# NJU-3DV/Relightable3DGaussian

Measured on AMD Instinct MI355X. Metric: train iters/s, synthetic lego-like 800x800, 300000 Gaussians (stage-2 hot path), higher is better.
Workload: dtype f32; 1 GPU; stage-2 train iteration (fused glue kernels + one-launch Adam): shading fwd/bwd (K=64) + rasterize fwd (S=16) + loss + rasterize bwd + Adam; 1 view/rank/step, 300000 Gaussians, 800x800, num_rendered~1755024; parallelism=dp1

## Files before the change

### relightable3dgaussian_amd/csrc/capi_shading.hip

```cpp
#include "capi_internal.hpp"

using namespace r3dg;

extern "C" {

int r3dg_shade_forward_cached(void* stream_, int P, int K, int M, const float* base_color, const float* roughness,
                              const float* normals, const float* viewdirs, const float* incidents, const float* env,
                              int He, int We, const float* env_transform, const float* visibility,
                              const float* incident_dirs, const float* incident_areas, float uniform_area,
                              const uint32_t* taps, int flags, float* out)
{
    if (P < 0 || K <= 0 || He <= 0 || We <= 0) return invalid("shade_forward: bad P/K/env size");
    if (He > 32767 || We > 32767) return invalid("shade_forward: environment map larger than 32767 texels per side");
    if (M != 1 && M != 4 && M != 9 && M != 16) return invalid("shade_forward: incidents must hold 1, 4, 9 or 16 SH coefficients");
    if (P == 0) return R3DG_OK;
    if (!base_color || !roughness || !normals || !viewdirs || !incidents || !env || !visibility || !incident_dirs || !out)
        return invalid("shade_forward: null buffer");
    return guarded([&]() -> int {
        hipStream_t stream = (hipStream_t)stream_;
        StageTimer t(stream, ST_SHADE_FWD);
        launch_shade_forward(stream, P, K, M, base_color, roughness, normals, viewdirs, incidents, env, He, We,
                             env_transform, visibility, incident_dirs, incident_areas, out, taps,
                             (flags & R3DG_SHADE_TRAIN_OUTPUTS) != 0, uniform_area, (flags & R3DG_SHADE_TAPS_ARE_RADIANCE) != 0,
                             (flags & R3DG_SHADE_LEAVE_ROOM) != 0);
// ... 239 lines not shown
    if (!shade_frs_supported(K, 16, He, We))
        return invalid("shade_frs_backward: needs K % 4 == 0 and an environment texture that fits LDS (r3dg_shade_frs_supported)");
    if (P == 0) return R3DG_OK;
    if (!base_color || !roughness || !normals || !viewdirs || !incidents || !env || !visibility || !taps || !ray_normals ||
        !zsamples || !tables || !valid || !cprime || !dcprime || !dL_dpbr || !dL_ddiffuse_light || !dL_dbase_color ||
        !dL_droughness || !dL_dviewdirs || !dL_dincidents || !dL_denv || (n_invalid > 0 && !invalid_list))
        return invalid("shade_frs_backward: null buffer");
    return guarded([&]() -> int {
        hipStream_t stream = (hipStream_t)stream_;
        int gmax_n = 1;
        const unsigned int* gmax;
        {
            StageTimer t(stream, ST_SHADE_AUX);
            gmax = launch_shade_frs_backward_aux(stream, P, dL_dpbr, dL_ddiffuse_light, block_absmax, n_block_absmax, &gmax_n);
        }
        if (n_invalid > 0) {
            StageTimer t(stream, ST_SHADE_LISTED);
            launch_shade_frs_backward_listed(stream, K, base_color, roughness, normals, viewdirs, incidents, env, He, We,
                                             visibility, ray_normals, zsamples, uniform_area, invalid_list, n_invalid, dL_dpbr,
                                             dL_ddiffuse_light, dL_dbase_color, dL_droughness, dL_dviewdirs, dL_dincidents,
                                             dL_denv, gmax, gmax_n);
        }
        {
            StageTimer t(stream, ST_SHADE_BWD);
            launch_shade_frs_backward_main(stream, P, K, base_color, roughness, normals, viewdirs, env, He, We, visibility,
                                           uniform_area, taps, ray_normals, tables, valid, cprime, dcprime, dL_dpbr,
                                           dL_ddiffuse_light, dL_dbase_color, dL_droughness, dL_dviewdirs, dL_denv, gmax, gmax_n);
        }
        if (no_rotation_back) return R3DG_OK;
        hipStream_t rstream = rotate_stream_ != nullptr ? (hipStream_t)rotate_stream_ : stream;
        stream_wait_stream(rstream, stream);
        {
            StageTimer t(rstream, ST_SHADE_AUX);
            launch_shade_frs_backward_rotate(rstream, P, ray_normals, dcprime, dL_dincidents, n_invalid > 0 ? valid : nullptr);
        }
        return R3DG_OK;
    });
}

int r3dg_shade_frs_incident_chain(void* stream_, int P, const float* ray_normals, const uint8_t* valid, const float* dcprime,
                                  float* dL_dincidents, float* incidents, float* exp_avg, float* exp_avg_sq, float* cprime,
                                  float lr, float lr_tail, float beta1, float beta2, float eps, int step, float grad_scale,
// ... 100 lines not shown
```

### relightable3dgaussian_amd/csrc/launchers.hpp

```cpp
#pragma once
#include "common.hpp"

namespace r3dg {

constexpr int REFILL_MIN_IDLE = 16;

void release_gradient_records();
void launch_mark_visible(hipStream_t s, int P, const float* means3D, const float* vm, uint8_t* present);
void launch_preprocess(hipStream_t s, int P, int D, int M, const float* means3D, const float* scales, float scale_modifier,
                       const float* rotations, const float* opacities, const float* shs, uint8_t* clamped,
                       const float* cov3D_precomp, const float* colors_precomp, const float* vm, const float* pm,
                       const float* cam_pos, int W, int H, float tan_fovx, float tan_fovy, float focal_x, float focal_y,
                       int* radii, float* means2D, float* depths, float* cov3Ds, float* rgb, float* conic_opacity,
                       float* splat, int gx, int gy, uint32_t* tiles_touched, uint32_t* block_sums,
                       unsigned long long* total, bool scan_now, uint32_t* zero_words, int zero_n);
void launch_duplicate_with_keys(hipStream_t s, int P, const float* means2D, const float* depths,
                                const uint32_t* tiles_touched, const uint32_t* block_offsets, uint32_t* point_offsets,
                                uint64_t* keys, uint32_t* values, const int* radii, int gx, int gy);
void launch_identify_tile_ranges(hipStream_t s, int L, const uint64_t* keys, uint32_t* ranges);
void launch_tile_order(hipStream_t s, int T, const uint32_t* ranges, uint32_t* order, uint32_t small_cap, uint32_t* big_list,
                       uint32_t* big_count);
void launch_render_forward(hipStream_t s, int W, int H, int S, const uint32_t* tile_order, const uint32_t* ranges,
                           const uint32_t* point_list, const float* splat, const float* features, float* final_T,
                           uint32_t* n_contrib, const float* bg, float* out_color, float* out_opacity, float* out_depth,
// ... 33 lines not shown
                                   const float* visibility, float uniform_area, const uint32_t* taps,
                                   const float* ray_normals, const float* tables, const uint8_t* valid, const float* cprime,
                                   bool leave_room, float* out, float* feat);
void launch_shade_frs_forward_listed(hipStream_t s, int K, const float* base_color, const float* roughness,
                                     const float* normals, const float* viewdirs, const float* incidents, const float* env,
                                     int He, int We, const float* visibility, const float* ray_normals,
                                     const float* zsamples, float uniform_area, const int* invalid_list, int n_invalid,
                                     float* out, float* feat);
void launch_shade_frs_incident_chain(hipStream_t s, int P, const float* ray_normals, const uint8_t* valid, const float* dcp,
                                     float* d_inc, float* incidents, float* exp_avg, float* exp_avg_sq, float* cprime,
                                     float lr, float lr_tail, float beta1, float beta2, float eps, int step,
                                     float grad_scale, const float* skip_flag, int listed_in_dcprime);
const unsigned int* launch_shade_frs_backward_aux(hipStream_t s, int P, const float* g_pbr, const float* g_diff,
                                                  const float* block_absmax, int n_block_absmax, int* gmax_n);
void launch_shade_frs_backward_main(hipStream_t s, int P, int K, const float* base_color, const float* roughness,
                                    const float* normals, const float* viewdirs, const float* env, int He, int We,
                                    const float* visibility, float uniform_area, const uint32_t* taps,
                                    const float* ray_normals, const float* tables, const uint8_t* valid, const float* cprime,
                                    float* dcp, const float* g_pbr, const float* g_diff, float* d_base, float* d_rough,
                                    float* d_view, float* d_env, const unsigned int* gmax, int gmax_n);
void launch_shade_frs_backward_rotate(hipStream_t s, int P, const float* ray_normals, const float* dcp, float* d_inc,
                                      const uint8_t* valid);
void launch_shade_frs_backward_listed(hipStream_t s, int K, const float* base_color, const float* roughness,
                                      const float* normals, const float* viewdirs, const float* incidents, const float* env,
                                      int He, int We, const float* visibility, const float* ray_normals,
                                      const float* zsamples, float uniform_area, const int* invalid_list, int n_invalid,
                                      const float* g_pbr, const float* g_diff, float* d_base, float* d_rough, float* d_view,
                                      float* d_inc, float* d_env, const unsigned int* gmax, int gmax_n);
void launch_shade_build_taps(hipStream_t s, size_t n, const float* dirs, const float* tr, int He, int We, const float* env,
                             uint32_t* taps);
void launch_shade_build_split(hipStream_t s, int P, int K, const int* perm, const float* normals, const float* incidents,
                              const float* visibility, const float* dirs, const float* zsamples, float uniform_area,
                              float* lt, float* vis_t, float* consts);
void launch_shade_forward_split(hipStream_t s, int P, int K, const int* perm, const float* base_color,
                                const float* roughness, const float* normals, const float* viewdirs, const float* lt,
                                const float* vis_t, const float* consts, const float* zsamples, const float* tr,
                                const float* env4, int He, int We, float* out);
void launch_shade_env_footprints(hipStream_t s, int He, int We, const float* env, float* fp);
void launch_shade_build_transport(hipStream_t s, int P, int K, int M, const float* normals, const float* incidents,
                                  const float* visibility, const float* dirs, const float* areas, float uniform_area,
                                  float* radiance_to_transport, float* consts);
void launch_shade_forward_transport(hipStream_t s, int P, int K, const float* base_color, const float* roughness,
                                    const float* normals, const float* viewdirs, const float* transport, const float* consts,
// ... 123 lines not shown
```

### relightable3dgaussian_amd/csrc/shading.hip

```cpp
#include "launchers.hpp"
#include <cmath>
#include <cstdlib>
#include <map>
#include <mutex>
#include <stdexcept>
#include <tuple>
#include "wave_reduce.hpp"
#include "shading_math.hpp"

namespace r3dg {

constexpr int SHADE_WAVES = 4;
constexpr int ENV_LDS_MAX = 12288;

__device__ __forceinline__ float fast_acosf(float x)
{
    const float ax = fabsf(x);
    const bool big = ax > 0.5f;
    const float z = big ? 0.5f * (1.0f - ax) : x * x;
    const float s = big ? sqrtf(z) : ax;
    float p = 4.2163199048e-2f;
    p = p * z + 2.4181311049e-2f;
    p = p * z + 4.5470025998e-2f;
    p = p * z + 7.4953002686e-2f;
// ... 100 lines not shown
            o.idx[a * 2 + b] = ok ? __mul24(y, We) + x : -1;
            o.w[a * 2 + b] = wy[a] * wx[b];
        }
    return o;
}

struct SampleFwd {
    float local[3], glob[3], lin[3], transport[3];
    float spec, ndi, area_ndi;
    float Y[16], shsum[3];
    float L[3], Hh[3], ulen, NoL, NoH, VoH, rawNoH, rawVoH, nom0, nom1, nom2, nomr, frac0, p2;
    EnvTap taps;
    float vis;
};

template <bool ENV_LDS, bool HAVE_SHSUM = false, bool HAVE_TAP = false>
__device__ __forceinline__ void shade_sample(SampleFwd& s, const GaussFwd& G, const float* sh ,
                                             int M, float dx, float dy, float dz, float vis, float area,
                                             const float* __restrict__ env, const float* s_env,
                                             const float* __restrict__ tr, int He, int We, const PackedTap* cached = nullptr)
{
    if (HAVE_TAP) s.taps = taps_from_packed(*cached, He, We);
    else s.taps = env_taps(dx, dy, dz, tr, He, We);
    s.vis = vis;
    float e[3] = {0.f, 0.f, 0.f};
#pragma unroll
    for (int t = 0; t < 4; t++) {
        if (s.taps.idx[t] >= 0) {
            float3 px;
            if (ENV_LDS) {
                const float* q = s_env + 3 * s.taps.idx[t];
                px = make_float3(q[0], q[1], q[2]);
            } else {
                px = *reinterpret_cast<const float3*>(env + 3 * (size_t)s.taps.idx[t]);
            }
            e[0] += px.x * s.taps.w[t];
            e[1] += px.y * s.taps.w[t];
            e[2] += px.z * s.taps.w[t];
        }
    }
    {
        float acc[3];
        if (HAVE_SHSUM) {
            acc[0] = s.shsum[0]; acc[1] = s.shsum[1]; acc[2] = s.shsum[2];
        } else {
            sh_basis16(dx, dy, dz, M, s.Y);
// ... 947 lines not shown
{
    unsigned int* scratch = shade_scratch();
    const unsigned int* gmax = scratch;
    *gmax_n = 1;
    if (block_absmax != nullptr && n_block_absmax > 0) {
        gmax = reinterpret_cast<const unsigned int*>(block_absmax);
        *gmax_n = n_block_absmax;
    } else {
        R3DG_HIP(hipMemsetAsync(scratch, 0, 4, s));
        const int nb = (3 * P + 255) / 256;
        grad_absmax_kernel<<<nb < 256 ? nb : 256, 256, 0, s>>>(3 * P, g_pbr, g_diff, scratch);
    }
    return gmax;
}

void launch_shade_frs_backward_main(hipStream_t s, int P, int K, const float* base_color, const float* roughness,
                                    const float* normals, const float* viewdirs, const float* env, int He, int We,
                                    const float* visibility, float uniform_area, const uint32_t* taps, const float* ray_normals,
                                    const float* tables, const uint8_t* valid, const float* cprime, float* dcp, const float* g_pbr,
                                    const float* g_diff, float* d_base, float* d_rough, float* d_view, float* d_env,
                                    const unsigned int* gmax, int gmax_n)
{
    if (P == 0) return;
    const bool tab_lds = K <= FRS_TAB_LDS_MAX_K;
    const size_t smem = frs_backward_lds_bytes(K, He, We);
    const FrsSrc src = {base_color, roughness, normals, viewdirs, ray_normals, cprime, g_pbr, g_diff, visibility, taps};
    if (tab_lds) {
        const int grid = frs_grid(P, (const void*)shade_backward_frs_kernel<true>, smem);
        shade_backward_frs_kernel<true><<<grid, 64 * FRS_WAVES, smem, s>>>(
            P, K, src, env, He, We, frs_area(uniform_area), tables, valid, d_base, d_rough, d_view, dcp, d_env, gmax, gmax_n);
    } else {
        const int grid = frs_grid(P, (const void*)shade_backward_frs_kernel<false>, smem);
        shade_backward_frs_kernel<false><<<grid, 64 * FRS_WAVES, smem, s>>>(
            P, K, src, env, He, We, frs_area(uniform_area), tables, valid, d_base, d_rough, d_view, dcp, d_env, gmax, gmax_n);
    }
    check_launch(s, false, "shade_backward_frs_kernel");
}

void launch_shade_frs_backward_rotate(hipStream_t s, int P, const float* ray_normals, const float* dcp, float* d_inc,
                                      const uint8_t* valid)
{
    if (P == 0) return;
    frs_rotate_kernel<true><<<(P + 255) / 256, 256, 0, s>>>(P, ray_normals, dcp, d_inc, valid);
    check_launch(s, false, "frs_rotate_kernel");
}

void launch_shade_frs_incident_chain(hipStream_t s, int P, const float* ray_normals, const uint8_t* valid, const float* dcp,
                                     float* d_inc, float* incidents, float* exp_avg, float* exp_avg_sq, float* cprime, float lr,
                                     float lr_tail, float beta1, float beta2, float eps, int step, float grad_scale,
                                     const float* skip_flag, int listed_in_dcprime)
{
    if (P == 0) return;
    const double b1 = 1.0 - pow((double)beta1, (double)step), b2 = 1.0 - pow((double)beta2, (double)step);
    FrsAdam a = {lr, lr_tail, beta1, beta2, eps, (float)b1, (float)(1.0 / sqrt(b2)), grad_scale, 1.f - beta1, 1.f - beta2};
    const size_t lds = 4 * 64 * FRS_CHAIN_LD * sizeof(float);
    frs_incident_chain_kernel<<<(P + 255) / 256, 256, lds, s>>>(P, ray_normals, valid, dcp, d_inc, incidents, exp_avg, exp_avg_sq,
                                                                cprime, a, skip_flag, listed_in_dcprime);
    check_launch(s, false, "frs_incident_chain_kernel");
}

void launch_shade_frs_backward_listed(hipStream_t s, int K, const float* base_color, const float* roughness,
                                      const float* normals, const float* viewdirs, const float* incidents, const float* env, int He,
                                      int We, const float* visibility, const float* ray_normals, const float* zsamples,
                                      float uniform_area, const int* invalid_list, int n_invalid, const float* g_pbr,
                                      const float* g_diff, float* d_base, float* d_rough, float* d_view, float* d_inc, float* d_env,
                                      const unsigned int* gmax, int gmax_n)
{
    if (n_invalid <= 0) return;
    const FrsSrc src = {base_color, roughness, normals, viewdirs, ray_normals, nullptr, g_pbr, g_diff, visibility, nullptr};
    const size_t smem = (3 * (((size_t)3 * He * We + 3) & ~(size_t)3) + 64 * FRS_LISTED_WAVES) * sizeof(float);
    int grid = frs_listed_grid(n_invalid);
    grid = grid > 64 ? 64 + (grid - 64) / 4 : grid;
    if (smem > 65536)
        R3DG_HIP(hipFuncSetAttribute((const void*)shade_backward_frs_listed_kernel, hipFuncAttributeMaxDynamicSharedMemorySize,
                                     (int)smem));
    shade_backward_frs_listed_kernel<<<grid, 64 * FRS_LISTED_WAVES, smem, s>>>(
        n_invalid, invalid_list, K, src, incidents, env, He, We, zsamples, frs_area(uniform_area), d_base, d_rough, d_view, d_inc,
        d_env, gmax, gmax_n);
    check_launch(s, false, "shade_backward_frs_listed_kernel");
}

void launch_shade_build_split(hipStream_t s, int P, int K, const int* perm, const float* normals, const float* incidents,
                              const float* visibility, const float* dirs, const float* zsamples, float uniform_area, float* lt,
                              float* vis_t, float* consts)
{
    if (P == 0) return;
    shade_build_split_kernel<<<(P + 255) / 256, 256, 0, s>>>(P, K, perm, normals, incidents, visibility, dirs, zsamples,
                                                           frs_area(uniform_area), reinterpret_cast<float4*>(lt), vis_t, consts);
    check_launch(s, false, "shade_build_split_kernel");
}

void launch_shade_forward_split(hipStream_t s, int P, int K, const int* perm, const float* base_color, const float* roughness,
                                const float* normals, const float* viewdirs, const float* lt, const float* vis_t,
                                const float* consts, const float* zsamples, const float* tr, const float* env_fp, int He, int We,
// ... 47 lines not shown
```

### relightable3dgaussian_amd/csrc/shading_frs.hpp

```cpp
#pragma once
#include "sh_rotation_tables.hpp"

namespace r3dg {

typedef float f32x4 __attribute__((ext_vector_type(4)));

constexpr int FRS_WAVES = 4;
constexpr int FRS_G = 16;
constexpr float FRS_MAX_DEFECT = 2e-5f;
constexpr int FRS_TAB_LDS_MAX_K = 128;

__device__ __forceinline__ void frs_rotation(const float n0, const float n1, const float n2, float (&R)[9])
{
    const float v1 = -n1, v2 = n0, cp = fmaxf(n2 + 1.f, 1e-7f);
    const bool regular = n2 + 1.f > 0.f;
    R[0] = regular ? 1.f + (-v2 * v2) / cp : -1.f;
    R[1] = regular ? v1 * v2 / cp : 0.f;
    R[2] = regular ? v2 : 0.f;
    R[3] = R[1];
    R[4] = regular ? 1.f + (-v1 * v1) / cp : -1.f;
    R[5] = regular ? -v1 : 0.f;
    R[6] = regular ? -v2 : 0.f;
    R[7] = regular ? v1 : 0.f;
    R[8] = regular ? 1.f + (-v2 * v2 - v1 * v1) / cp : -1.f;
// ... 563 lines not shown
        for (int i = 0; i < 7; i++) acc[i] = frs_sum4(acc[i]) * invK;
        if (live_g && q == 0) {
            float* o = out + (size_t)g * SHADE_NOUT;
#pragma unroll
            for (int i = 0; i < 6; i++) o[i] = acc[i];
            o[18] = acc[6];
            if (feat != nullptr) {
                float* f = feat + (size_t)g * 16;
                f[2] = acc[0]; f[3] = acc[1]; f[4] = acc[2];
                *reinterpret_cast<float4*>(f + 12) = make_float4(acc[3], acc[4], acc[5], acc[6]);
            }
        }
    }
}

template <bool TAB_LDS>
__global__ void __launch_bounds__(64 * FRS_WAVES, 2)
shade_backward_frs_kernel(int P, int K, FrsSrc src, const float* __restrict__ env , int He, int We,
                          float uniform_area, const float* __restrict__ tables, const uint8_t* __restrict__ valid,
                          float* __restrict__ d_base, float* __restrict__ d_rough, float* __restrict__ d_view,
                          float* __restrict__ dcp, float* __restrict__ d_env, const unsigned int* __restrict__ gmax_bits,
                          int gmax_n)
{
    extern __shared__ __attribute__((aligned(16))) float s_mem[];
    const int ntexel = He * We;
    float4* s_env4 = reinterpret_cast<float4*>(s_mem);
    long long* s_denv = reinterpret_cast<long long*>(s_mem + 4 * ntexel);
    const unsigned int gmax_word = wave_gmax_bits(gmax_bits, gmax_n);
    const float gmax = __uint_as_float(gmax_word);
    const bool fixed = gmax_usable(gmax_word);
    const float fx_scale = fixed ? 34359738368.0f / gmax : 0.f;
    const float fx_clamp = gmax * 8192.0f;
    const int nblk = (K + 15) >> 4;
    float* s_stage = s_mem + ((10 * ntexel + 3) & ~3);
    float* s_tab = s_stage + FRS_WAVES * FRS_ST_BWD;
    frs_stage_texture(env, ntexel, s_env4);
    for (int i = threadIdx.x; i < 3 * ntexel; i += blockDim.x) s_denv[i] = 0;
    if (TAB_LDS)
        for (int i = threadIdx.x; i < nblk * 512; i += blockDim.x) s_tab[i] = tables[i];
    __syncthreads();
    const int lane = threadIdx.x & 63, wave = threadIdx.x >> 6;
    const int gl = lane & 15, q = lane >> 4;
    const float invK = 1.0f / (float)K;
    const int ngroups = (P + FRS_G - 1) / FRS_G;
    float* st = s_stage + wave * FRS_ST_BWD;
    const unsigned int st_addr = lds_address_of(st);
    const int gstride = gridDim.x * FRS_WAVES;
    int grp = blockIdx.x * FRS_WAVES + wave;
    uint8_t nvalid = 0;
    if (grp < ngroups) {
        nvalid = valid[min(grp * FRS_G + gl, P - 1)];
        frs_stage_group<true>(st_addr, grp, P, K, lane, src);
    }
    for (; grp < ngroups; grp += gstride) {
        const int g = grp * FRS_G + gl;
        const int gc = min(g, P - 1);
        const bool live_g = g < P && nvalid != 0;
        asm volatile("s_waitcnt vmcnt(0)" ::: "memory");
        float u[64];
#pragma unroll
        for (int c = 0; c < 3; c++) {
            u[48 + c] = st[FRS_ST_BASE + 3 * gl + c];
            u[52 + c] = st[FRS_ST_NRM + 3 * gl + c];
            u[55 + c] = st[FRS_ST_VIEW + 3 * gl + c];
        }
        u[51] = st[FRS_ST_RGH + gl];
        const float rn0 = st[FRS_ST_RNRM + 3 * gl], rn1 = st[FRS_ST_RNRM + 3 * gl + 1], rn2 = st[FRS_ST_RNRM + 3 * gl + 2];
        const float gp[3] = {st[FRS_ST_GP + 3 * gl] * invK, st[FRS_ST_GP + 3 * gl + 1] * invK, st[FRS_ST_GP + 3 * gl + 2] * invK};
        const float gd[3] = {st[FRS_ST_GD + 3 * gl] * invK, st[FRS_ST_GD + 3 * gl + 1] * invK, st[FRS_ST_GD + 3 * gl + 2] * invK};
        float bc[4][3];
#pragma unroll
        for (int s = 0; s < 4; s++)
#pragma unroll
// ... 4 lines not shown
        FrsBlock nxt = frs_staged_block(st, gl, q, K);
        GaussFwd G;
        gauss_setup(G, u);
        FrsFrame F;
        {
            float R[9];
            frs_rotation(rn0, rn1, rn2, R);
            frs_frame(F, R, G.n[0], G.n[1], G.n[2], G.V[0], G.V[1], G.V[2], q);
        }
        const float fd[3] = {G.base[0] / kPi, G.base[1] / kPi, G.base[2] / kPi};
        const float nom1 = G.NoV * (1.f - G.kk) + G.kk;
        f32x4 dcq[3] = {{0.f, 0.f, 0.f, 0.f}, {0.f, 0.f, 0.f, 0.f}, {0.f, 0.f, 0.f, 0.f}};
        f32x4 dvq = {0.f, 0.f, 0.f, 0.f};
        float accb[5] = {0.f, 0.f, 0.f, 0.f, 0.f};
        const size_t row = (size_t)gc * (size_t)K;
        int ngrp_l = min(grp + gstride, ngroups - 1);
        int ngc_l = min(ngrp_l * FRS_G + gl, P - 1);
        for (int b = 0; b < nblk; b++) {
            const FrsBlock cur = nxt;
            const float* tb = (TAB_LDS ? s_tab : tables) + (size_t)b * 512 + lane;
            float a[4] = {0.f, 0.f, 0.f, 0.f}, a2[4] = {0.f, 0.f, 0.f, 0.f};
            if (!TAB_LDS) {
#pragma unroll
                for (int s = 0; s < 4; s++) {
                    a[s] = tb[64 * s];
                    a2[s] = tb[64 * (4 + s)];
                }
            }
            const bool last = b + 1 == nblk;
            if (!last) {
                nxt = frs_load_block(row, 16 * (b + 1) + 4 * q, K, src.visibility, src.taps);
            } else {
                asm volatile("" : "+v"(ngrp_l), "+v"(ngc_l));
                nvalid = valid[ngc_l];
            }
            __builtin_amdgcn_sched_barrier(0);
            if (TAB_LDS) {
#pragma unroll
                for (int s = 0; s < 4; s++) a[s] = tb[64 * s];
            }
            f32x4 l[3] = {{0.f, 0.f, 0.f, 0.f}, {0.f, 0.f, 0.f, 0.f}, {0.f, 0.f, 0.f, 0.f}};
#pragma unroll
            for (int s = 0; s < 4; s++)
#pragma unroll
                for (int c = 0; c < 3; c++) l[c] = __builtin_amdgcn_mfma_f32_16x16x4f32(a[s], bc[s][c], l[c], 0, 0, 0);
            const FrsGeom geo = frs_block_geometry(F, a[0], a[1], a[2]);
            if (last) frs_stage_group<true>(st_addr, ngrp_l, P, K, lane, src);
#pragma unroll
            for (int v = 0; v < 4; v++) {
// ... 97 lines not shown
#pragma unroll
                for (int m = 0; m < 3; m++) dV[m] = R[3 * m] * cx + R[3 * m + 1] * cy + R[3 * m + 2] * cz + accb[4] * G.N[m];
                const float vd = G.V[0] * dV[0] + G.V[1] * dV[1] + G.V[2] * dV[2];
#pragma unroll
                for (int c = 0; c < 3; c++) {
                    d_base[3 * (size_t)g + c] = accb[c];
                    d_view[3 * (size_t)g + c] = (dV[c] - G.V[c] * vd) / G.vlen;
                }
                d_rough[g] = accb[3];
            }
            float4* o = reinterpret_cast<float4*>(dcp + (size_t)g * 48 + 12 * q);
            o[0] = make_float4(dcq[0][0], dcq[1][0], dcq[2][0], dcq[0][1]);
            o[1] = make_float4(dcq[1][1], dcq[2][1], dcq[0][2], dcq[1][2]);
            o[2] = make_float4(dcq[2][2], dcq[0][3], dcq[1][3], dcq[2][3]);
        }
    }
    if (fixed) {
        __syncthreads();
        const float inv = 1.0f / fx_scale;
        for (int i = threadIdx.x; i < 3 * ntexel; i += blockDim.x) {
            const long long v64 = s_denv[i];
            if (v64 != 0) atomicAdd(&d_env[i], (float)((double)v64 * (double)inv));
        }
    }
}

constexpr int FRS_LISTED_WAVES = 4;

__device__ __forceinline__ float frs_listed_record(int lane, int g, const FrsSrc& p, const float* __restrict__ incidents)
{
    const float* q = incidents + (size_t)g * 48 + lane;
    if (lane >= 48) q = p.base_color + 3 * (size_t)g + (lane - 48);
    if (lane == 51) q = p.roughness + g;
    if (lane >= 52) q = p.normals + 3 * (size_t)g + (lane - 52);
    if (lane >= 55) q = p.viewdirs + 3 * (size_t)g + (lane - 55);
    if (lane >= 58) q = p.ray_normals + 3 * (size_t)g + (lane - 58);
    return lane < 61 ? *q : 0.f;
}

__device__ __forceinline__ void frs_listed_direction(const float (&R)[9], const float* __restrict__ zsamples, int k, float& dx,
                                                     float& dy, float& dz)
{
    const float zx = zsamples[3 * k], zy = zsamples[3 * k + 1], zz = zsamples[3 * k + 2];
    dx = R[0] * zx + R[1] * zy + R[2] * zz; dy = R[3] * zx + R[4] * zy + R[5] * zz; dz = R[6] * zx + R[7] * zy + R[8] * zz;
    const float len = fmaxf(sqrtf(dx * dx + dy * dy + dz * dz), 1e-12f);
    dx /= len; dy /= len; dz /= len;
}

__global__ void __launch_bounds__(64 * FRS_LISTED_WAVES)
shade_forward_frs_listed_kernel(int n_list, const int* __restrict__ list, int K, FrsSrc src,
                                const float* __restrict__ incidents, const float* __restrict__ env, int He, int We,
                                const float* __restrict__ zsamples, float uniform_area, float* __restrict__ out,
                                float* __restrict__ feat)
{
    extern __shared__ __attribute__((aligned(16))) float s_mem[];
    float* s_env = s_mem;
    const int ntex = 3 * He * We;
    for (int i = threadIdx.x; i < ntex; i += blockDim.x) s_env[i] = env[i];
    __syncthreads();
    const int lane = threadIdx.x & 63, wave = threadIdx.x >> 6;
    float* u = s_mem + ((ntex + 3) & ~3) + wave * 64;
// ... 19 lines not shown
                    v[c] += (G.base[c] / kPi + s.spec) * s.transport[c];
                    v[3 + c] += s.transport[c];
                }
                v[6] += vis;
            }
        }
        const float r = transpose_reduce<8, true>(v);
        const int ch = transposed_channel<8>(lane);
        if (transposed_owner<8>(lane) && ch < 7) {
            out[(size_t)g * SHADE_NOUT + (ch < 6 ? ch : 18)] = r * invK;
            if (feat != nullptr) feat[(size_t)g * 16 + (ch < 3 ? 2 + ch : 9 + ch)] = r * invK;
        }
    }
}

__global__ void __launch_bounds__(64 * FRS_LISTED_WAVES)
shade_backward_frs_listed_kernel(int n_list, const int* __restrict__ list, int K, FrsSrc src,
                                 const float* __restrict__ incidents, const float* __restrict__ env, int He, int We,
                                 const float* __restrict__ zsamples, float uniform_area, float* __restrict__ d_base,
                                 float* __restrict__ d_rough, float* __restrict__ d_view, float* __restrict__ d_inc,
                                 float* __restrict__ d_env, const unsigned int* __restrict__ gmax_bits, int gmax_n)
{
    extern __shared__ __attribute__((aligned(16))) float s_mem[];
    const int ntex = 3 * He * We, ntex4 = (ntex + 3) & ~3;
    float* s_env = s_mem;
    long long* s_denv = reinterpret_cast<long long*>(s_mem + ntex4);
    const unsigned int gmax_word = wave_gmax_bits(gmax_bits, gmax_n);
    const float gmax = __uint_as_float(gmax_word);
    const bool fixed = gmax_usable(gmax_word);
    const float fx_scale = fixed ? 34359738368.0f / gmax : 0.f;
    const float fx_clamp = gmax * 8192.0f;
    for (int i = threadIdx.x; i < ntex; i += blockDim.x) {
        s_env[i] = env[i];
        s_denv[i] = 0;
    }
    __syncthreads();
    const int lane = threadIdx.x & 63, wave = threadIdx.x >> 6;
    float* u = s_mem + 3 * ntex4 + wave * 64;
    const float invK = 1.0f / (float)K;
    for (int i = blockIdx.x * FRS_LISTED_WAVES + wave; i < n_list; i += gridDim.x * FRS_LISTED_WAVES) {
        const int g = __builtin_amdgcn_readfirstlane(list[i]);
        u[lane] = frs_listed_record(lane, g, src, incidents);
        GaussFwd G;
        gauss_setup(G, u);
        float R[9];
        frs_rotation(u[58], u[59], u[60], R);
        float gp[3], gd[3];
#pragma unroll
        for (int c = 0; c < 3; c++) {
            gp[c] = src.g_pbr[3 * (size_t)g + c] * invK;
            gd[c] = src.g_diff[3 * (size_t)g + c] * invK;
        }
        float acc[64];
#pragma unroll
        for (int f = 0; f < 64; f++) acc[f] = 0.f;
        for (int kb = 0; kb < K; kb += 64) {
            const int k = kb + lane, kc = min(k, K - 1);
            float dx, dy, dz;
            frs_listed_direction(R, zsamples, kc, dx, dy, dz);
            const float vis = src.visibility[(size_t)g * K + kc];
            SampleFwd s;
            shade_sample<true>(s, G, u, 16, dx, dy, dz, vis, k < K ? uniform_area : 0.f, nullptr, s_env, nullptr, He, We);
            float gspec = 0.f, dlin[3], dl[3];
#pragma unroll
            for (int c = 0; c < 3; c++) {
                const float dT = gp[c] * (G.base[c] / kPi + s.spec) + gd[c];
                gspec += gp[c] * s.transport[c];
                acc[48 + c] += gp[c] * s.transport[c] / kPi;
                dlin[c] = dT * s.area_ndi;
                dl[c] = s.shsum[c] >= 0.f ? dlin[c] : 0.f;
            }
            if (s.vis != 0.f && s.area_ndi != 0.f) {
                const float ev[3] = {dlin[0] * s.vis, dlin[1] * s.vis, dlin[2] * s.vis};
                const double scale_d = (double)fx_scale;
#pragma unroll
                for (int tt = 0; tt < 4; tt++) {
                    if (s.taps.idx[tt] < 0) continue;
#pragma unroll
                    for (int c = 0; c < 3; c++) {
                        const float val = ev[c] * s.taps.w[tt];
                        if (fixed) {
                            const float cl = __builtin_amdgcn_fmed3f(val, -fx_clamp, fx_clamp);
                            const double dsum = __builtin_fma((double)cl, scale_d, 6755399441055744.0);
                            const unsigned long long bits = (unsigned long long)__double_as_longlong(dsum) - 0x4338000000000000ull;
                            atomicAdd(reinterpret_cast<unsigned long long*>(&s_denv[3 * s.taps.idx[tt] + c]), bits);
                        } else {
                            atomicAdd(&d_env[3 * (size_t)s.taps.idx[tt] + c], val);
                        }
                    }
                }
            }
            const float frac = s.frac0 * G.a2;
            const bool nom_free = s.nomr >= 1e-6f && s.nomr <= 4.f * kPi;
            const float nom = fminf(fmaxf(s.nomr, 1e-6f), 4.f * kPi);
            const float dfrac = gspec / nom;
            const float dnom = nom_free ? -gspec * frac / (nom * nom) : 0.f;
            float da2 = dfrac * s.frac0;
            const float dFMi = dfrac * G.a2 * 0.96f * 0.6931471805599453f * s.p2;
            float dVoH = dFMi * (-2.f * 5.55473f * s.VoH - 6.98316f);
            const float c4 = 4.f * kPi;
            const float dnom0 = dnom * c4 * 2.f * s.nom0 * s.nom1 * s.nom2;
            const float dnom1 = dnom * c4 * s.nom0 * s.nom0 * s.nom2;
            const float dnom2 = dnom * c4 * s.nom0 * s.nom0 * s.nom1;
            float dNoH = dnom0 * 2.f * s.NoH * (G.a2 - 1.f);
            da2 += dnom0 * s.NoH * s.NoH;
            float dNoV = dnom1 * (1.f - G.kk);
            const float dkk = dnom1 * (1.f - G.NoV) + dnom2 * (1.f - s.NoL);
            const float da = dkk / 8.f + da2 * 2.f * G.a;
            acc[51] += dkk * 2.f / 8.f + da * 2.f * G.r;
            if (!(s.rawNoH >= 1e-6f && s.rawNoH <= 1.f)) dNoH = 0.f;
            if (!(s.rawVoH >= 1e-6f && s.rawVoH <= 1.f)) dVoH = 0.f;
            if (!(G.rawNoV >= 1e-6f && G.rawNoV <= 1.f)) dNoV = 0.f;
            float dH[3], dV[3];
#pragma unroll
            for (int c = 0; c < 3; c++) {
                dH[c] = dNoH * G.N[c] + dVoH * G.V[c];
                dV[c] = dVoH * s.Hh[c] + dNoV * G.N[c];
            }
            const float hd = s.Hh[0] * dH[0] + s.Hh[1] * dH[1] + s.Hh[2] * dH[2];
#pragma unroll
            for (int c = 0; c < 3; c++) dV[c] += 0.5f * (dH[c] - s.Hh[c] * hd) / s.ulen;
            const float vd = G.V[0] * dV[0] + G.V[1] * dV[1] + G.V[2] * dV[2];
#pragma unroll
            for (int c = 0; c < 3; c++) acc[52 + c] += (dV[c] - G.V[c] * vd) / G.vlen;
#pragma unroll
            for (int f = 0; f < 48; f++) acc[f] += dl[f % 3] * s.Y[f / 3];
        }
        const float r = transpose_reduce<64, true>(acc);
        const int ch = transposed_channel<64>(lane);
        if (ch < 48) d_inc[(size_t)g * 48 + ch] = r;
        else if (ch < 51) d_base[3 * (size_t)g + (ch - 48)] = r;
        else if (ch == 51) d_rough[g] = r;
        else if (ch < 55) d_view[3 * (size_t)g + (ch - 52)] = r;
    }
    if (fixed) {
        __syncthreads();
        const float inv = 1.0f / fx_scale;
        for (int i = threadIdx.x; i < ntex; i += blockDim.x) {
            const long long v64 = s_denv[i];
            if (v64 != 0) atomicAdd(&d_env[i], (float)((double)v64 * (double)inv));
        }
    }
}

}
```

Baseline: 812.2 iters/s.

## Fold listed-invalid shading backward into main FRS backward kernel with ticket scheduling

Removes the separate listed-Gaussian backward kernel and processes invalid-listed Gaussians inside the main FRS backward kernel. A global atomic ticket counter hands out groups dynamically after a first static pass, and the counter is reset by the last block to finish. Listed work reuses the main kernel's LDS environment copy, read with a stride of 4, so the environment texture is not staged twice and one launch is saved. The cost is a more complex persistent kernel, a per-stream ticket buffer, and possible extra register or LDS pressure in the main kernel.

```diff
diff --git a/relightable3dgaussian_amd/csrc/capi_shading.hip b/relightable3dgaussian_amd/csrc/capi_shading.hip
--- a/relightable3dgaussian_amd/csrc/capi_shading.hip
+++ b/relightable3dgaussian_amd/csrc/capi_shading.hip
@@ -277,18 +277,12 @@
             StageTimer t(stream, ST_SHADE_AUX);
             gmax = launch_shade_frs_backward_aux(stream, P, dL_dpbr, dL_ddiffuse_light, block_absmax, n_block_absmax, &gmax_n);
         }
-        if (n_invalid > 0) {
-            StageTimer t(stream, ST_SHADE_LISTED);
-            launch_shade_frs_backward_listed(stream, K, base_color, roughness, normals, viewdirs, incidents, env, He, We,
-                                             visibility, ray_normals, zsamples, uniform_area, invalid_list, n_invalid, dL_dpbr,
-                                             dL_ddiffuse_light, dL_dbase_color, dL_droughness, dL_dviewdirs, dL_dincidents,
-                                             dL_denv, gmax, gmax_n);
-        }
         {
             StageTimer t(stream, ST_SHADE_BWD);
-            launch_shade_frs_backward_main(stream, P, K, base_color, roughness, normals, viewdirs, env, He, We, visibility,
-                                           uniform_area, taps, ray_normals, tables, valid, cprime, dcprime, dL_dpbr,
-                                           dL_ddiffuse_light, dL_dbase_color, dL_droughness, dL_dviewdirs, dL_denv, gmax, gmax_n);
+            launch_shade_frs_backward_main(stream, P, K, base_color, roughness, normals, viewdirs, incidents, env, He, We,
+                                           visibility, uniform_area, taps, ray_normals, zsamples, tables, valid, invalid_list,
+                                           n_invalid, cprime, dcprime, dL_dpbr, dL_ddiffuse_light, dL_dbase_color, dL_droughness,
+                                           dL_dviewdirs, dL_dincidents, dL_denv, gmax, gmax_n);
         }
         if (no_rotation_back) return R3DG_OK;
         hipStream_t rstream = rotate_stream_ != nullptr ? (hipStream_t)rotate_stream_ : stream;
diff --git a/relightable3dgaussian_amd/csrc/launchers.hpp b/relightable3dgaussian_amd/csrc/launchers.hpp
--- a/relightable3dgaussian_amd/csrc/launchers.hpp
+++ b/relightable3dgaussian_amd/csrc/launchers.hpp
@@ -71,19 +71,14 @@
 const unsigned int* launch_shade_frs_backward_aux(hipStream_t s, int P, const float* g_pbr, const float* g_diff,
                                                   const float* block_absmax, int n_block_absmax, int* gmax_n);
 void launch_shade_frs_backward_main(hipStream_t s, int P, int K, const float* base_color, const float* roughness,
-                                    const float* normals, const float* viewdirs, const float* env, int He, int We,
-                                    const float* visibility, float uniform_area, const uint32_t* taps,
-                                    const float* ray_normals, const float* tables, const uint8_t* valid, const float* cprime,
-                                    float* dcp, const float* g_pbr, const float* g_diff, float* d_base, float* d_rough,
-                                    float* d_view, float* d_env, const unsigned int* gmax, int gmax_n);
+                                    const float* normals, const float* viewdirs, const float* incidents, const float* env, int He,
+                                    int We, const float* visibility, float uniform_area, const uint32_t* taps,
+                                    const float* ray_normals, const float* zsamples, const float* tables, const uint8_t* valid,
+                                    const int* invalid_list, int n_invalid, const float* cprime, float* dcp, const float* g_pbr,
+                                    const float* g_diff, float* d_base, float* d_rough, float* d_view, float* d_inc_listed,
+                                    float* d_env, const unsigned int* gmax, int gmax_n);
 void launch_shade_frs_backward_rotate(hipStream_t s, int P, const float* ray_normals, const float* dcp, float* d_inc,
                                       const uint8_t* valid);
-void launch_shade_frs_backward_listed(hipStream_t s, int K, const float* base_color, const float* roughness,
-                                      const float* normals, const float* viewdirs, const float* incidents, const float* env,
-                                      int He, int We, const float* visibility, const float* ray_normals,
-                                      const float* zsamples, float uniform_area, const int* invalid_list, int n_invalid,
-                                      const float* g_pbr, const float* g_diff, float* d_base, float* d_rough, float* d_view,
-                                      float* d_inc, float* d_env, const unsigned int* gmax, int gmax_n);
 void launch_shade_build_taps(hipStream_t s, size_t n, const float* dirs, const float* tr, int He, int We, const float* env,
                              uint32_t* taps);
 void launch_shade_build_split(hipStream_t s, int P, int K, const int* perm, const float* normals, const float* incidents,
diff --git a/relightable3dgaussian_amd/csrc/shading.hip b/relightable3dgaussian_amd/csrc/shading.hip
--- a/relightable3dgaussian_amd/csrc/shading.hip
+++ b/relightable3dgaussian_amd/csrc/shading.hip
@@ -138,7 +138,7 @@
     float vis;
 };
 
-template <bool ENV_LDS, bool HAVE_SHSUM = false, bool HAVE_TAP = false>
+template <bool ENV_LDS, bool HAVE_SHSUM = false, bool HAVE_TAP = false, int ENV_STRIDE = 3>
 __device__ __forceinline__ void shade_sample(SampleFwd& s, const GaussFwd& G, const float* sh ,
                                              int M, float dx, float dy, float dz, float vis, float area,
                                              const float* __restrict__ env, const float* s_env,
@@ -153,7 +153,7 @@
         if (s.taps.idx[t] >= 0) {
             float3 px;
             if (ENV_LDS) {
-                const float* q = s_env + 3 * s.taps.idx[t];
+                const float* q = s_env + ENV_STRIDE * s.taps.idx[t];
                 px = make_float3(q[0], q[1], q[2]);
             } else {
                 px = *reinterpret_cast<const float3*>(env + 3 * (size_t)s.taps.idx[t]);
@@ -1131,26 +1131,47 @@
     return gmax;
 }
 
+static unsigned int* frs_ticket_words(hipStream_t s)
+{
+    static std::mutex mu;
+    static std::map<std::pair<int, hipStream_t>, unsigned int*> words;
+    int dev = 0;
+    R3DG_HIP(hipGetDevice(&dev));
+    std::lock_guard<std::mutex> lk(mu);
+    unsigned int*& p = words[std::make_pair(dev, s)];
+    if (p == nullptr) {
+        R3DG_HIP(hipMalloc((void**)&p, 64));
+        R3DG_HIP(hipMemset(p, 0, 64));
+    }
+    return p;
+}
+
 void launch_shade_frs_backward_main(hipStream_t s, int P, int K, const float* base_color, const float* roughness,
-                                    const float* normals, const float* viewdirs, const float* env, int He, int We,
-                                    const float* visibility, float uniform_area, const uint32_t* taps, const float* ray_normals,
-                                    const float* tables, const uint8_t* valid, const float* cprime, float* dcp, const float* g_pbr,
-                                    const float* g_diff, float* d_base, float* d_rough, float* d_view, float* d_env,
-                                    const unsigned int* gmax, int gmax_n)
+                                    const float* normals, const float* viewdirs, const float* incidents, const float* env, int He,
+                                    int We, const float* visibility, float uniform_area, const uint32_t* taps,
+                                    const float* ray_normals, const float* zsamples, const float* tables, const uint8_t* valid,
+                                    const int* invalid_list, int n_invalid, const float* cprime, float* dcp, const float* g_pbr,
+                                    const float* g_diff, float* d_base, float* d_rough, float* d_view, float* d_inc_listed,
+                                    float* d_env, const unsigned int* gmax, int gmax_n)
 {
     if (P == 0) return;
     const bool tab_lds = K <= FRS_TAB_LDS_MAX_K;
     const size_t smem = frs_backward_lds_bytes(K, He, We);
     const FrsSrc src = {base_color, roughness, normals, viewdirs, ray_normals, cprime, g_pbr, g_diff, visibility, taps};
-    if (tab_lds) {
-        const int grid = frs_grid(P, (const void*)shade_backward_frs_kernel<true>, smem);
+    const void* kernel = tab_lds ? (const void*)shade_backward_frs_kernel<true> : (const void*)shade_backward_frs_kernel<false>;
+    const int grid = frs_grid(P, kernel, smem);
+    const int ngroups = (P + FRS_G - 1) / FRS_G, nblk = (K + 15) / 16;
+    const int chunk = nblk >= 8 ? 1 : 8 / nblk;
+    const int n_single = ngroups < grid * FRS_WAVES ? ngroups : grid * FRS_WAVES;
+    const FrsTickets tk = {frs_ticket_words(s), chunk, (ngroups - n_single) / chunk, invalid_list, n_invalid > 0 ? n_invalid : 0};
+    if (tab_lds)
         shade_backward_frs_kernel<true><<<grid, 64 * FRS_WAVES, smem, s>>>(
-            P, K, src, env, He, We, frs_area(uniform_area), tables, valid, d_base, d_rough, d_view, dcp, d_env, gmax, gmax_n);
-    } else {
-        const int grid = frs_grid(P, (const void*)shade_backward_frs_kernel<false>, smem);
+            P, K, src, env, He, We, frs_area(uniform_area), tables, valid, d_base, d_rough, d_view, dcp, d_env, gmax, gmax_n, tk,
+            incidents, zsamples, d_inc_listed);
+    else
         shade_backward_frs_kernel<false><<<grid, 64 * FRS_WAVES, smem, s>>>(
-            P, K, src, env, He, We, frs_area(uniform_area), tables, valid, d_base, d_rough, d_view, dcp, d_env, gmax, gmax_n);
-    }
+            P, K, src, env, He, We, frs_area(uniform_area), tables, valid, d_base, d_rough, d_view, dcp, d_env, gmax, gmax_n, tk,
+            incidents, zsamples, d_inc_listed);
     check_launch(s, false, "shade_backward_frs_kernel");
 }
 
@@ -1174,27 +1195,6 @@
     frs_incident_chain_kernel<<<(P + 255) / 256, 256, lds, s>>>(P, ray_normals, valid, dcp, d_inc, incidents, exp_avg, exp_avg_sq,
                                                                 cprime, a, skip_flag, listed_in_dcprime);
     check_launch(s, false, "frs_incident_chain_kernel");
-}
-
-void launch_shade_frs_backward_listed(hipStream_t s, int K, const float* base_color, const float* roughness,
-                                      const float* normals, const float* viewdirs, const float* incidents, const float* env, int He,
-                                      int We, const float* visibility, const float* ray_normals, const float* zsamples,
-                                      float uniform_area, const int* invalid_list, int n_invalid, const float* g_pbr,
-                                      const float* g_diff, float* d_base, float* d_rough, float* d_view, float* d_inc, float* d_env,
-                                      const unsigned int* gmax, int gmax_n)
-{
-    if (n_invalid <= 0) return;
-    const FrsSrc src = {base_color, roughness, normals, viewdirs, ray_normals, nullptr, g_pbr, g_diff, visibility, nullptr};
-    const size_t smem = (3 * (((size_t)3 * He * We + 3) & ~(size_t)3) + 64 * FRS_LISTED_WAVES) * sizeof(float);
-    int grid = frs_listed_grid(n_invalid);
-    grid = grid > 64 ? 64 + (grid - 64) / 4 : grid;
-    if (smem > 65536)
-        R3DG_HIP(hipFuncSetAttribute((const void*)shade_backward_frs_listed_kernel, hipFuncAttributeMaxDynamicSharedMemorySize,
-                                     (int)smem));
-    shade_backward_frs_listed_kernel<<<grid, 64 * FRS_LISTED_WAVES, smem, s>>>(
-        n_invalid, invalid_list, K, src, incidents, env, He, We, zsamples, frs_area(uniform_area), d_base, d_rough, d_view, d_inc,
-        d_env, gmax, gmax_n);
-    check_launch(s, false, "shade_backward_frs_listed_kernel");
 }
 
 void launch_shade_build_split(hipStream_t s, int P, int K, const int* perm, const float* normals, const float* incidents,
diff --git a/relightable3dgaussian_amd/csrc/shading_frs.hpp b/relightable3dgaussian_amd/csrc/shading_frs.hpp
--- a/relightable3dgaussian_amd/csrc/shading_frs.hpp
+++ b/relightable3dgaussian_amd/csrc/shading_frs.hpp
@@ -601,13 +601,160 @@
     }
 }
 
+constexpr int FRS_LISTED_WAVES = 4;
+
+__device__ __forceinline__ float frs_listed_record(int lane, int g, const FrsSrc& p, const float* __restrict__ incidents)
+{
+    const float* q = incidents + (size_t)g * 48 + lane;
+    if (lane >= 48) q = p.base_color + 3 * (size_t)g + (lane - 48);
+    if (lane == 51) q = p.roughness + g;
+    if (lane >= 52) q = p.normals + 3 * (size_t)g + (lane - 52);
+    if (lane >= 55) q = p.viewdirs + 3 * (size_t)g + (lane - 55);
+    if (lane >= 58) q = p.ray_normals + 3 * (size_t)g + (lane - 58);
+    return lane < 61 ? *q : 0.f;
+}
+
+__device__ __forceinline__ void frs_listed_direction(const float (&R)[9], const float* __restrict__ zsamples, int k, float& dx,
+                                                     float& dy, float& dz)
+{
+    const float zx = zsamples[3 * k], zy = zsamples[3 * k + 1], zz = zsamples[3 * k + 2];
+    dx = R[0] * zx + R[1] * zy + R[2] * zz; dy = R[3] * zx + R[4] * zy + R[5] * zz; dz = R[6] * zx + R[7] * zy + R[8] * zz;
+    const float len = fmaxf(sqrtf(dx * dx + dy * dy + dz * dz), 1e-12f);
+    dx /= len; dy /= len; dz /= len;
+}
+
+__device__ __forceinline__ void frs_listed_backward(int g, int K, int lane, const FrsSrc& src, const float* __restrict__ incidents,
+                                                    const float* s_env4, int He, int We, const float* __restrict__ zsamples,
+                                                    float uniform_area, float* u, long long* s_denv, bool fixed, float fx_scale,
+                                                    float fx_clamp, float* __restrict__ d_base, float* __restrict__ d_rough,
+                                                    float* __restrict__ d_view, float* __restrict__ d_inc,
+                                                    float* __restrict__ d_env)
+{
+    const float invK = 1.0f / (float)K;
+    u[lane] = frs_listed_record(lane, g, src, incidents);
+    GaussFwd G;
+    gauss_setup(G, u);
+    float R[9];
+    frs_rotation(u[58], u[59], u[60], R);
+    float gp[3], gd[3];
+#pragma unroll
+    for (int c = 0; c < 3; c++) {
+        gp[c] = src.g_pbr[3 * (size_t)g + c] * invK;
+        gd[c] = src.g_diff[3 * (size_t)g + c] * invK;
+    }
+    float acc[64];
+#pragma unroll
+    for (int f = 0; f < 64; f++) acc[f] = 0.f;
+    for (int kb = 0; kb < K; kb += 64) {
+        const int k = kb + lane, kc = min(k, K - 1);
+        float dx, dy, dz;
+        frs_listed_direction(R, zsamples, kc, dx, dy, dz);
+        const float vis = src.visibility[(size_t)g * K + kc];
+        SampleFwd s;
+        shade_sample<true, false, false, 4>(s, G, u, 16, dx, dy, dz, vis, k < K ? uniform_area : 0.f, nullptr, s_env4, nullptr,
+                                            He, We);
+        float gspec = 0.f, dlin[3], dl[3];
+#pragma unroll
+        for (int c = 0; c < 3; c++) {
+            const float dT = gp[c] * (G.base[c] / kPi + s.spec) + gd[c];
+            gspec += gp[c] * s.transport[c];
+            acc[48 + c] += gp[c] * s.transport[c] / kPi;
+            dlin[c] = dT * s.area_ndi;
+            dl[c] = s.shsum[c] >= 0.f ? dlin[c] : 0.f;
+        }
+        if (s.vis != 0.f && s.area_ndi != 0.f) {
+            const float ev[3] = {dlin[0] * s.vis, dlin[1] * s.vis, dlin[2] * s.vis};
+            const double scale_d = (double)fx_scale;
+#pragma unroll
+            for (int tt = 0; tt < 4; tt++) {
+                if (s.taps.idx[tt] < 0) continue;
+#pragma unroll
+                for (int c = 0; c < 3; c++) {
+                    const float val = ev[c] * s.taps.w[tt];
+                    if (fixed) {
+                        const float cl = __builtin_amdgcn_fmed3f(val, -fx_clamp, fx_clamp);
+                        const double dsum = __builtin_fma((double)cl, scale_d, 6755399441055744.0);
+                        const unsigned long long bits = (unsigned long long)__double_as_longlong(dsum) - 0x4338000000000000ull;
+                        atomicAdd(reinterpret_cast<unsigned long long*>(&s_denv[3 * s.taps.idx[tt] + c]), bits);
+                    } else {
+                        atomicAdd(&d_env[3 * (size_t)s.taps.idx[tt] + c], val);
+                    }
+                }
+            }
+        }
+        const float frac = s.frac0 * G.a2;
+        const bool nom_free = s.nomr >= 1e-6f && s.nomr <= 4.f * kPi;
+        const float nom = fminf(fmaxf(s.nomr, 1e-6f), 4.f * kPi);
+        const float dfrac = gspec / nom;
+        const float dnom = nom_free ? -gspec * frac / (nom * nom) : 0.f;
+        float da2 = dfrac * s.frac0;
+        const float dFMi = dfrac * G.a2 * 0.96f * 0.6931471805599453f * s.p2;
+        float dVoH = dFMi * (-2.f * 5.55473f * s.VoH - 6.98316f);
+        const float c4 = 4.f * kPi;
+        const float dnom0 = dnom * c4 * 2.f * s.nom0 * s.nom1 * s.nom2;
+        const float dnom1 = dnom * c4 * s.nom0 * s.nom0 * s.nom2;
+        const float dnom2 = dnom * c4 * s.nom0 * s.nom0 * s.nom1;
+        float dNoH = dnom0 * 2.f * s.NoH * (G.a2 - 1.f);
+        da2 += dnom0 * s.NoH * s.NoH;
+        float dNoV = dnom1 * (1.f - G.kk);
+        const float dkk = dnom1 * (1.f - G.NoV) + dnom2 * (1.f - s.NoL);
+        const float da = dkk / 8.f + da2 * 2.f * G.a;
+        acc[51] += dkk * 2.f / 8.f + da * 2.f * G.r;
+        if (!(s.rawNoH >= 1e-6f && s.rawNoH <= 1.f)) dNoH = 0.f;
+        if (!(s.rawVoH >= 1e-6f && s.rawVoH <= 1.f)) dVoH = 0.f;
+        if (!(G.rawNoV >= 1e-6f && G.rawNoV <= 1.f)) dNoV = 0.f;
+        float dH[3], dV[3];
+#pragma unroll
+        for (int c = 0; c < 3; c++) {
+            dH[c] = dNoH * G.N[c] + dVoH * G.V[c];
+            dV[c] = dVoH * s.Hh[c] + dNoV * G.N[c];
+        }
+        const float hd = s.Hh[0] * dH[0] + s.Hh[1] * dH[1] + s.Hh[2] * dH[2];
+#pragma unroll
+        for (int c = 0; c < 3; c++) dV[c] += 0.5f * (dH[c] - s.Hh[c] * hd) / s.ulen;
+        const float vd = G.V[0] * dV[0] + G.V[1] * dV[1] + G.V[2] * dV[2];
+#pragma unroll
+        for (int c = 0; c < 3; c++) acc[52 + c] += (dV[c] - G.V[c] * vd) / G.vlen;
+#pragma unroll
+        for (int f = 0; f < 48; f++) acc[f] += dl[f % 3] * s.Y[f / 3];
+    }
+    const float r = transpose_reduce<64, true>(acc);
+    const int ch = transposed_channel<64>(lane);
+    if (ch < 48) d_inc[(size_t)g * 48 + ch] = r;
+    else if (ch < 51) d_base[3 * (size_t)g + (ch - 48)] = r;
+    else if (ch == 51) d_rough[g] = r;
+    else if (ch < 55) d_view[3 * (size_t)g + (ch - 52)] = r;
+}
+
+struct FrsTickets {
+    unsigned int* words;
+    int chunk, n_chunked;
+    const int* list;
+    int n_list;
+};
+
+__device__ __forceinline__ int frs_ticket_first(const FrsTickets& tk, int t, int& count)
+{
+    const bool chunked = t < tk.n_chunked;
+    count = chunked ? tk.chunk : 1;
+    return chunked ? t * tk.chunk : tk.n_chunked * (tk.chunk - 1) + t;
+}
+
+__device__ __forceinline__ unsigned int frs_draw(const FrsTickets& tk, int lane)
+{
+    unsigned int v = 0;
+    if (lane == 0) v = __hip_atomic_fetch_add(tk.words, 1u, __ATOMIC_RELAXED, __HIP_MEMORY_SCOPE_AGENT);
+    return v;
+}
+
 template <bool TAB_LDS>
 __global__ void __launch_bounds__(64 * FRS_WAVES, 2)
 shade_backward_frs_kernel(int P, int K, FrsSrc src, const float* __restrict__ env , int He, int We,
                           float uniform_area, const float* __restrict__ tables, const uint8_t* __restrict__ valid,
                           float* __restrict__ d_base, float* __restrict__ d_rough, float* __restrict__ d_view,
                           float* __restrict__ dcp, float* __restrict__ d_env, const unsigned int* __restrict__ gmax_bits,
-                          int gmax_n)
+                          int gmax_n, FrsTickets tk, const float* __restrict__ incidents, const float* __restrict__ zsamples,
+                          float* __restrict__ d_inc_listed )
 {
     extern __shared__ __attribute__((aligned(16))) float s_mem[];
     const int ntexel = He * We;
@@ -626,24 +773,29 @@
     if (TAB_LDS)
         for (int i = threadIdx.x; i < nblk * 512; i += blockDim.x) s_tab[i] = tables[i];
     __syncthreads();
-    const int lane = threadIdx.x & 63, wave = threadIdx.x >> 6;
+    const int lane = threadIdx.x & 63, wave = __builtin_amdgcn_readfirstlane(threadIdx.x >> 6);
     const int gl = lane & 15, q = lane >> 4;
     const float invK = 1.0f / (float)K;
     const int ngroups = (P + FRS_G - 1) / FRS_G;
     float* st = s_stage + wave * FRS_ST_BWD;
     const unsigned int st_addr = lds_address_of(st);
-    const int gstride = gridDim.x * FRS_WAVES;
-    int grp = blockIdx.x * FRS_WAVES + wave;
+    const int nstatic = gridDim.x * FRS_WAVES;
+    int rem;
+    int grp = frs_ticket_first(tk, blockIdx.x * FRS_WAVES + wave, rem);
+    rem -= 1;
     uint8_t nvalid = 0;
     if (grp < ngroups) {
         nvalid = valid[min(grp * FRS_G + gl, P - 1)];
         frs_stage_group<true>(st_addr, grp, P, K, lane, src);
     }
-    for (; grp < ngroups; grp += gstride) {
+    while (grp < ngroups) {
         const int g = grp * FRS_G + gl;
         const int gc = min(g, P - 1);
         const bool live_g = g < P && nvalid != 0;
         asm volatile("s_waitcnt vmcnt(0)" ::: "memory");
+        unsigned int drawn = 0;
+        if (rem == 0) drawn = frs_draw(tk, lane);
+        int nxt_grp = grp + 1, nxt_rem = rem - 1;
         float u[64];
 #pragma unroll
         for (int c = 0; c < 3; c++) {
@@ -678,8 +830,7 @@
         f32x4 dvq = {0.f, 0.f, 0.f, 0.f};
         float accb[5] = {0.f, 0.f, 0.f, 0.f, 0.f};
         const size_t row = (size_t)gc * (size_t)K;
-        int ngrp_l = min(grp + gstride, ngroups - 1);
-        int ngc_l = min(ngrp_l * FRS_G + gl, P - 1);
+        int ngrp_l = ngroups - 1;
         for (int b = 0; b < nblk; b++) {
             const FrsBlock cur = nxt;
             const float* tb = (TAB_LDS ? s_tab : tables) + (size_t)b * 512 + lane;
@@ -695,8 +846,13 @@
             if (!last) {
                 nxt = frs_load_block(row, 16 * (b + 1) + 4 * q, K, src.visibility, src.taps);
             } else {
-                asm volatile("" : "+v"(ngrp_l), "+v"(ngc_l));
-                nvalid = valid[ngc_l];
+                if (rem == 0) {
+                    const int t = nstatic + (int)__builtin_amdgcn_readfirstlane(drawn);
+                    nxt_grp = frs_ticket_first(tk, t, nxt_rem);
+                    nxt_rem -= 1;
+                }
+                ngrp_l = min(nxt_grp, ngroups - 1);
+                nvalid = valid[min(ngrp_l * FRS_G + gl, P - 1)];
             }
             __builtin_amdgcn_sched_barrier(0);
             if (TAB_LDS) {
@@ -824,37 +980,33 @@
             o[1] = make_float4(dcq[1][1], dcq[2][1], dcq[0][2], dcq[1][2]);
             o[2] = make_float4(dcq[2][2], dcq[0][3], dcq[1][3], dcq[2][3]);
         }
+        grp = nxt_grp;
+        rem = nxt_rem;
+    }
+    asm volatile("s_waitcnt vmcnt(0)" ::: "memory");
+    const int nwork = ngroups + tk.n_list;
+    while (grp < nwork) {
+        const unsigned int drawn = frs_draw(tk, lane);
+        const int g = __builtin_amdgcn_readfirstlane(tk.list[grp - ngroups]);
+        frs_listed_backward(g, K, lane, src, incidents, reinterpret_cast<const float*>(s_env4), He, We, zsamples, uniform_area,
+                            st, s_denv, fixed, fx_scale, fx_clamp, d_base, d_rough, d_view, d_inc_listed, d_env);
+        grp = frs_ticket_first(tk, nstatic + (int)__builtin_amdgcn_readfirstlane(drawn), rem);
+    }
+    __syncthreads();
+    if (threadIdx.x == 0) {
+        const unsigned int done = __hip_atomic_fetch_add(tk.words + 1, 1u, __ATOMIC_RELAXED, __HIP_MEMORY_SCOPE_AGENT);
+        if (done == gridDim.x - 1) {
+            __hip_atomic_store(tk.words, 0u, __ATOMIC_RELAXED, __HIP_MEMORY_SCOPE_AGENT);
+            __hip_atomic_store(tk.words + 1, 0u, __ATOMIC_RELAXED, __HIP_MEMORY_SCOPE_AGENT);
+        }
     }
     if (fixed) {
-        __syncthreads();
         const float inv = 1.0f / fx_scale;
         for (int i = threadIdx.x; i < 3 * ntexel; i += blockDim.x) {
             const long long v64 = s_denv[i];
             if (v64 != 0) atomicAdd(&d_env[i], (float)((double)v64 * (double)inv));
         }
     }
-}
-
-constexpr int FRS_LISTED_WAVES = 4;
-
-__device__ __forceinline__ float frs_listed_record(int lane, int g, const FrsSrc& p, const float* __restrict__ incidents)
-{
-    const float* q = incidents + (size_t)g * 48 + lane;
-    if (lane >= 48) q = p.base_color + 3 * (size_t)g + (lane - 48);
-    if (lane == 51) q = p.roughness + g;
-    if (lane >= 52) q = p.normals + 3 * (size_t)g + (lane - 52);
-    if (lane >= 55) q = p.viewdirs + 3 * (size_t)g + (lane - 55);
-    if (lane >= 58) q = p.ray_normals + 3 * (size_t)g + (lane - 58);
-    return lane < 61 ? *q : 0.f;
-}
-
-__device__ __forceinline__ void frs_listed_direction(const float (&R)[9], const float* __restrict__ zsamples, int k, float& dx,
-                                                     float& dy, float& dz)
-{
-    const float zx = zsamples[3 * k], zy = zsamples[3 * k + 1], zz = zsamples[3 * k + 2];
-    dx = R[0] * zx + R[1] * zy + R[2] * zz; dy = R[3] * zx + R[4] * zy + R[5] * zz; dz = R[6] * zx + R[7] * zy + R[8] * zz;
-    const float len = fmaxf(sqrtf(dx * dx + dy * dy + dz * dz), 1e-12f);
-    dx /= len; dy /= len; dz /= len;
 }
 
 __global__ void __launch_bounds__(64 * FRS_LISTED_WAVES)
@@ -904,133 +1056,4 @@
     }
 }
 
-__global__ void __launch_bounds__(64 * FRS_LISTED_WAVES)
-shade_backward_frs_listed_kernel(int n_list, const int* __restrict__ list, int K, FrsSrc src,
-                                 const float* __restrict__ incidents, const float* __restrict__ env, int He, int We,
-                                 const float* __restrict__ zsamples, float uniform_area, float* __restrict__ d_base,
-                                 float* __restrict__ d_rough, float* __restrict__ d_view, float* __restrict__ d_inc,
-                                 float* __restrict__ d_env, const unsigned int* __restrict__ gmax_bits, int gmax_n)
-{
-    extern __shared__ __attribute__((aligned(16))) float s_mem[];
-    const int ntex = 3 * He * We, ntex4 = (ntex + 3) & ~3;
-    float* s_env = s_mem;
-    long long* s_denv = reinterpret_cast<long long*>(s_mem + ntex4);
-    const unsigned int gmax_word = wave_gmax_bits(gmax_bits, gmax_n);
-    const float gmax = __uint_as_float(gmax_word);
-    const bool fixed = gmax_usable(gmax_word);
-    const float fx_scale = fixed ? 34359738368.0f / gmax : 0.f;
-    const float fx_clamp = gmax * 8192.0f;
-    for (int i = threadIdx.x; i < ntex; i += blockDim.x) {
-        s_env[i] = env[i];
-        s_denv[i] = 0;
-    }
-    __syncthreads();
-    const int lane = threadIdx.x & 63, wave = threadIdx.x >> 6;
-    float* u = s_mem + 3 * ntex4 + wave * 64;
-    const float invK = 1.0f / (float)K;
-    for (int i = blockIdx.x * FRS_LISTED_WAVES + wave; i < n_list; i += gridDim.x * FRS_LISTED_WAVES) {
-        const int g = __builtin_amdgcn_readfirstlane(list[i]);
-        u[lane] = frs_listed_record(lane, g, src, incidents);
-        GaussFwd G;
-        gauss_setup(G, u);
-        float R[9];
-        frs_rotation(u[58], u[59], u[60], R);
-        float gp[3], gd[3];
-#pragma unroll
-        for (int c = 0; c < 3; c++) {
-            gp[c] = src.g_pbr[3 * (size_t)g + c] * invK;
-            gd[c] = src.g_diff[3 * (size_t)g + c] * invK;
-        }
-        float acc[64];
-#pragma unroll
-        for (int f = 0; f < 64; f++) acc[f] = 0.f;
-        for (int kb = 0; kb < K; kb += 64) {
-            const int k = kb + lane, kc = min(k, K - 1);
-            float dx, dy, dz;
-            frs_listed_direction(R, zsamples, kc, dx, dy, dz);
-            const float vis = src.visibility[(size_t)g * K + kc];
-            SampleFwd s;
-            shade_sample<true>(s, G, u, 16, dx, dy, dz, vis, k < K ? uniform_area : 0.f, nullptr, s_env, nullptr, He, We);
-            float gspec = 0.f, dlin[3], dl[3];
-#pragma unroll
-            for (int c = 0; c < 3; c++) {
-                const float dT = gp[c] * (G.base[c] / kPi + s.spec) + gd[c];
-                gspec += gp[c] * s.transport[c];
-                acc[48 + c] += gp[c] * s.transport[c] / kPi;
-                dlin[c] = dT * s.area_ndi;
-                dl[c] = s.shsum[c] >= 0.f ? dlin[c] : 0.f;
-            }
-            if (s.vis != 0.f && s.area_ndi != 0.f) {
-                const float ev[3] = {dlin[0] * s.vis, dlin[1] * s.vis, dlin[2] * s.vis};
-                const double scale_d = (double)fx_scale;
-#pragma unroll
-                for (int tt = 0; tt < 4; tt++) {
-                    if (s.taps.idx[tt] < 0) continue;
-#pragma unroll
-                    for (int c = 0; c < 3; c++) {
-                        const float val = ev[c] * s.taps.w[tt];
-                        if (fixed) {
-                            const float cl = __builtin_amdgcn_fmed3f(val, -fx_clamp, fx_clamp);
-                            const double dsum = __builtin_fma((double)cl, scale_d, 6755399441055744.0);
-                            const unsigned long long bits = (unsigned long long)__double_as_longlong(dsum) - 0x4338000000000000ull;
-                            atomicAdd(reinterpret_cast<unsigned long long*>(&s_denv[3 * s.taps.idx[tt] + c]), bits);
-                        } else {
-                            atomicAdd(&d_env[3 * (size_t)s.taps.idx[tt] + c], val);
-                        }
-                    }
-                }
-            }
-            const float frac = s.frac0 * G.a2;
-            const bool nom_free = s.nomr >= 1e-6f && s.nomr <= 4.f * kPi;
-            const float nom = fminf(fmaxf(s.nomr, 1e-6f), 4.f * kPi);
-            const float dfrac = gspec / nom;
-            const float dnom = nom_free ? -gspec * frac / (nom * nom) : 0.f;
-            float da2 = dfrac * s.frac0;
-            const float dFMi = dfrac * G.a2 * 0.96f * 0.6931471805599453f * s.p2;
-            float dVoH = dFMi * (-2.f * 5.55473f * s.VoH - 6.98316f);
-            const float c4 = 4.f * kPi;
-            const float dnom0 = dnom * c4 * 2.f * s.nom0 * s.nom1 * s.nom2;
-            const float dnom1 = dnom * c4 * s.nom0 * s.nom0 * s.nom2;
-            const float dnom2 = dnom * c4 * s.nom0 * s.nom0 * s.nom1;
-            float dNoH = dnom0 * 2.f * s.NoH * (G.a2 - 1.f);
-            da2 += dnom0 * s.NoH * s.NoH;
-            float dNoV = dnom1 * (1.f - G.kk);
-            const float dkk = dnom1 * (1.f - G.NoV) + dnom2 * (1.f - s.NoL);
-            const float da = dkk / 8.f + da2 * 2.f * G.a;
-            acc[51] += dkk * 2.f / 8.f + da * 2.f * G.r;
-            if (!(s.rawNoH >= 1e-6f && s.rawNoH <= 1.f)) dNoH = 0.f;
-            if (!(s.rawVoH >= 1e-6f && s.rawVoH <= 1.f)) dVoH = 0.f;
-            if (!(G.rawNoV >= 1e-6f && G.rawNoV <= 1.f)) dNoV = 0.f;
-            float dH[3], dV[3];
-#pragma unroll
-            for (int c = 0; c < 3; c++) {
-                dH[c] = dNoH * G.N[c] + dVoH * G.V[c];
-                dV[c] = dVoH * s.Hh[c] + dNoV * G.N[c];
-            }
-            const float hd = s.Hh[0] * dH[0] + s.Hh[1] * dH[1] + s.Hh[2] * dH[2];
-#pragma unroll
-            for (int c = 0; c < 3; c++) dV[c] += 0.5f * (dH[c] - s.Hh[c] * hd) / s.ulen;
-            const float vd = G.V[0] * dV[0] + G.V[1] * dV[1] + G.V[2] * dV[2];
-#pragma unroll
-            for (int c = 0; c < 3; c++) acc[52 + c] += (dV[c] - G.V[c] * vd) / G.vlen;
-#pragma unroll
-            for (int f = 0; f < 48; f++) acc[f] += dl[f % 3] * s.Y[f / 3];
-        }
-        const float r = transpose_reduce<64, true>(acc);
-        const int ch = transposed_channel<64>(lane);
-        if (ch < 48) d_inc[(size_t)g * 48 + ch] = r;
-        else if (ch < 51) d_base[3 * (size_t)g + (ch - 48)] = r;
-        else if (ch == 51) d_rough[g] = r;
-        else if (ch < 55) d_view[3 * (size_t)g + (ch - 52)] = r;
-    }
-    if (fixed) {
-        __syncthreads();
-        const float inv = 1.0f / fx_scale;
-        for (int i = threadIdx.x; i < ntex; i += blockDim.x) {
-            const long long v64 = s_denv[i];
-            if (v64 != 0) atomicAdd(&d_env[i], (float)((double)v64 * (double)inv));
-        }
-    }
-}
-
-}
+}
```

Result: no change. 806.9 iters/s (-0.6%).
